# daigo0927/tf-raft

Measured on AMD Instinct MI355X. Metric: image-pairs/sec at 448×512 iters_pred=24; final-iter EPE vs TF ref, higher is better.
Workload: dtype f32; 1 GPU; RAFT forward BASELINE configs[1]: batch 4/GPU 448x512 iters_pred=24 random weights; pairs_per_gpu=4, global_batch=4, parallelism=dp1, collective=none

## Files before the change

### tf_raft_amd/csrc/conv_halo.h

```cpp
#pragma once
#include <stdlib.h>
#include <type_traits>

#include "conv_mfma.h"

template <int KH, int KW, int TH, int TN, int EPI, int STRIDE = 1, int PRE = 0, int STATS = 0, int STEM = 0, int DEEP = 0>
__global__ void __launch_bounds__(256) conv_halo_kernel(ConvArgs p) {
    constexpr int TW = 16, NKK = 2;
    constexpr int TAPS = KH * KW, R = TAPS * NKK;
    constexpr int LSTEP = (TAPS == 1 && !STEM) ? STRIDE : 1;
    constexpr int FSTEP = (TAPS == 1) ? 1 : STRIDE;
    constexpr int LDA = (FSTEP == 2) ? 36 : 40;
    constexpr int HH = (TH - 1) * FSTEP + KH, HWP = (TW - 1) * FSTEP + KW, HP = HH * HWP;
    constexpr int NA = (HP * 8 + 255) / 256;
    constexpr int A_BUF = HP * LDA + 8;
    constexpr int BN = 64 * TN;
    static_assert(!STEM || (TAPS == 1 && STRIDE == 2 && !PRE), "stem mode: 1x1 addressing, stride 2");
    __shared__ __attribute__((aligned(16))) float smem[2 * A_BUF];

    const int tid = threadIdx.x, lane = tid & 63, wn = tid >> 6;
    const int G = lane >> 4, LR = lane & 15;
    const int tiles_x = (p.W + TW - 1) / TW, tiles_y = (p.H + TH - 1) / TH;
    const int ntn = p.npad / BN;
    const int M = p.B * p.H * p.W;
    const int Hi = p.Hi, Wi = p.Wi;
    const int Min = p.B * Hi * Wi;

    int bid = blockIdx.x;
    {
        const int nwg = gridDim.x, xcd = bid & 7, q = nwg >> 3, r = nwg & 7;
        bid = (xcd < r ? xcd * (q + 1) : r * (q + 1) + (xcd - r) * q) + (bid >> 3);
    }
    const int mt = bid / ntn, nt = bid - mt * ntn;
    const int tx = mt % tiles_x, ty = (mt / tiles_x) % tiles_y, b = mt / (tiles_x * tiles_y);
    const int y0 = ty * TH, x0 = tx * TW;
    const int n0 = nt * BN;
    const int cin = p.c0 + p.c1;
    const int nch = cin >> 5;

    const __amdgpu_buffer_rsrc_t rs0 = __builtin_amdgcn_make_buffer_rsrc(
        (void *)p.a0, 0, (int)((((long)Min - 1) * p.lda0 + (STEM ? 4 : p.c0)) * 4), 0x00020000);
    const __amdgpu_buffer_rsrc_t rs1 = __builtin_amdgcn_make_buffer_rsrc(
        (void *)(p.c1 ? p.a1 : p.a0), 0, p.c1 ? (int)((((long)Min - 1) * p.lda1 + p.c1) * 4) : 0, 0x00020000);
    const __amdgpu_buffer_rsrc_t rsw = __builtin_amdgcn_make_buffer_rsrc(
        (void *)p.wp, 0, (int)((long)TAPS * cin * p.npad * 4), 0x00020000);

    int pix[NA];
    int lds_off[NA];
#pragma unroll
    for (int i = 0; i < NA; ++i) {
        const int item = tid + 256 * i;
        const int hp = item >> 3, c4 = item & 7;
        const int hy = hp / HWP, hx = hp - hy * HWP;
        lds_off[i] = hp < HP ? hp * LDA + c4 * 4 : HP * LDA;
        if (STEM) {
            const int yy = (y0 + hy) * 2 - p.pt, xx = (x0 + hx) * 2 - p.pl + c4;
            const bool ok = (hp < HP) & (c4 < 7) & ((unsigned)xx < (unsigned)Wi);
            pix[i] = ok ? (b * Hi + yy) * Wi + xx : -(1 << 30);
        } else {
            const int yy = y0 * STRIDE - p.pt + hy * LSTEP, xx = x0 * STRIDE - p.pl + hx * LSTEP;
            const bool ok = (hp < HP) & ((unsigned)yy < (unsigned)Hi) & ((unsigned)xx < (unsigned)Wi);
            pix[i] = ok ? (b * Hi + yy) * Wi + xx : -1;
        }
    }
    f32x4 ra[NA], pre_sc, pre_sh;
    auto gload = [&](int c) {
        if (STEM) {
#pragma unroll
            for (int i = 0; i < NA; ++i) {
                const int hp = (tid + 256 * i) >> 3;
                const int yy = (y0 + hp / HWP) * 2 - p.pt + c;
                const bool ok = (pix[i] > -(1 << 29)) & ((unsigned)yy < (unsigned)Hi);
                ra[i] = raft_buffer_load_f4(rs0, ok ? (unsigned)((pix[i] + c * Wi) * 16) : RAFT_OOB);
            }
            return;
        }
        const int ch = c * 32;
        const bool first = ch < p.c0;
        const int ld = first ? p.lda0 : p.lda1;
        const int chl = (first ? ch : ch - p.c0) + (tid & 7) * 4;
        if (first) {
#pragma unroll
            for (int i = 0; i < NA; ++i)
                ra[i] = raft_buffer_load_f4(rs0, pix[i] >= 0 ? (unsigned)((pix[i] * ld + chl) * 4) : RAFT_OOB);
        } else {
#pragma unroll
            for (int i = 0; i < NA; ++i)
                ra[i] = raft_buffer_load_f4(rs1, pix[i] >= 0 ? (unsigned)((pix[i] * ld + chl) * 4) : RAFT_OOB);
        }
        if (PRE) {
            pre_sc = *(const f32x4 *)(p.pre_scale + (long)b * cin + ch + (tid & 7) * 4);
            pre_sh = *(const f32x4 *)(p.pre_shift + (long)b * cin + ch + (tid & 7) * 4);
        }
    };
    auto lstore = [&](int buf) {
#pragma unroll
        for (int i = 0; i < NA; ++i) {
            f32x4 v = ra[i];
            if (PRE) {
#pragma unroll
                for (int e = 0; e < 4; ++e) v[e] = pix[i] >= 0 ? fmaxf(fmaf(v[e], pre_sc[e], pre_sh[e]), 0.f) : 0.f;
            }
            *(f32x4 *)(smem + buf * A_BUF + lds_off[i]) = v;
        }
    };

    f32x4 fa[2][TH], fb[DEEP ? 4 : 2][TN];
    const int a_lane = LR * FSTEP * LDA + G * 4;
    const unsigned b_lane = (unsigned)(((G * p.npad) + n0 + wn * 16 * TN + LR) * 16);
    auto frag_a = [&](int buf, int q, f32x4 *a) {
        const int t = q / NKK, kk = q - t * NKK;
        const float *base = smem + buf * A_BUF + a_lane + ((t / KW) * HWP + (t % KW)) * LDA + kk * 16;
#pragma unroll
        for (int i = 0; i < TH; ++i) a[i] = *(const f32x4 *)(base + i * FSTEP * HWP * LDA);
    };
    auto frag_b = [&](int c, int q, f32x4 *bf) {
        const int t = q / NKK, kk = q - t * NKK;
        const unsigned row = (unsigned)((t * (cin >> 2) + c * 8 + kk * 4) * p.npad) * 16u;
#pragma unroll
        for (int j = 0; j < TN; ++j)
            bf[j] = __builtin_bit_cast(f32x4, __builtin_amdgcn_raw_buffer_load_b128(rsw, (int)(b_lane + j * 256), (int)row, 0));
    };

    f32x4 acc[TH][TN];
#pragma unroll
    for (int i = 0; i < TH; ++i)
#pragma unroll
        for (int j = 0; j < TN; ++j) acc[i][j] = f32x4{0.f, 0.f, 0.f, 0.f};

    const int w0 = (EPI == EPI_GRU_ZR) ? p.hid : p.nvalid;
    const int w1 = (EPI == EPI_GRU_ZR) ? p.nvalid - p.hid : 0;
    const __amdgpu_buffer_rsrc_t ro0 = __builtin_amdgcn_make_buffer_rsrc(
        (void *)p.o0, 0, (int)((((long)M - 1) * p.ldo0 + w0) * 4), 0x00020000);
    const __amdgpu_buffer_rsrc_t ro1 = __builtin_amdgcn_make_buffer_rsrc(
        (void *)(w1 > 0 ? p.o1 : p.o0), 0, w1 > 0 ? (int)((((long)M - 1) * p.ldo1 + w1) * 4) : 0, 0x00020000);
    const bool has_e0 = EPI == EPI_GRU_ZR || EPI == EPI_GRU_Q || EPI == EPI_RES, has_e1 = EPI == EPI_GRU_Q;
    const int we = (EPI == EPI_GRU_ZR) ? p.hid : p.nvalid;
    const __amdgpu_buffer_rsrc_t re0 = __builtin_amdgcn_make_buffer_rsrc(
        (void *)(has_e0 ? (const void *)p.e0 : (const void *)p.o0), 0,
        has_e0 ? (int)((((long)M - 1) * p.lde0 + we) * 4) : 0, 0x00020000);
    const __amdgpu_buffer_rsrc_t re1 = __builtin_amdgcn_make_buffer_rsrc(
        (void *)(has_e1 ? (const void *)p.e1 : (const void *)p.o0), 0,
        has_e1 ? (int)((((long)M - 1) * p.lde1 + we) * 4) : 0, 0x00020000);
    auto bstore = [](float v, __amdgpu_buffer_rsrc_t r, unsigned off) {
        __builtin_amdgcn_raw_buffer_store_b32(__builtin_bit_cast(unsigned, v), r, (int)off, 0, 0);
    };
    auto bload = [](__amdgpu_buffer_rsrc_t r, unsigned off) {
        return __builtin_bit_cast(float, __builtin_amdgcn_raw_buffer_load_b32(r, (int)off, 0, 0));
    };
    float pe0[TH][TN][4], pe1[TH][TN][4];
    if (EPI == EPI_RES || EPI == EPI_GRU_ZR || EPI == EPI_GRU_Q) {
#pragma unroll
        for (int i = 0; i < TH; ++i)
#pragma unroll
            for (int j = 0; j < TN; ++j) {
                const int n = n0 + (wn * TN + j) * 16 + LR;
                const bool nok = n < p.nvalid;
                const bool isz = n < p.hid;
                const unsigned ne = (EPI == EPI_GRU_ZR) ? (unsigned)(isz ? n : n - p.hid) : (unsigned)n;
                const bool want0 = (EPI == EPI_GRU_ZR) ? (nok & !isz) : nok;
#pragma unroll
                for (int r = 0; r < 4; ++r) {
                    const int yy = y0 + i, xx = x0 + 4 * G + r;
                    const bool mokr = (yy < p.H) & (xx < p.W);
                    const unsigned m = (unsigned)((b * p.H + yy) * p.W + xx);
                    pe0[i][j][r] = bload(re0, (want0 & mokr) ? (m * p.lde0 + ne) * 4u : RAFT_OOB);
                    if (EPI == EPI_GRU_Q) pe1[i][j][r] = bload(re1, (nok & mokr) ? (m * p.lde1 + n) * 4u : RAFT_OOB);
                }
            }
    }
    gload(0);
    frag_b(0, 0, fb[0]);
    if (p.init) {
        const __amdgpu_buffer_rsrc_t ri = __builtin_amdgcn_make_buffer_rsrc(
            (void *)p.init, 0, (int)((((long)M - 1) * p.ldi + p.nvalid) * 4), 0x00020000);
#pragma unroll
        for (int i = 0; i < TH; ++i)
#pragma unroll
            for (int j = 0; j < TN; ++j) {
                const int n = n0 + (wn * TN + j) * 16 + LR;
#pragma unroll
                for (int r = 0; r < 4; ++r) {
                    const int yy = y0 + i, xx = x0 + 4 * G + r;
                    const bool ok = (yy < p.H) & (xx < p.W) & (n < p.nvalid);
                    const unsigned m = (unsigned)((b * p.H + yy) * p.W + xx);
                    acc[i][j][r] = __builtin_bit_cast(
                        float, __builtin_amdgcn_raw_buffer_load_b32(ri, ok ? (int)((m * p.ldi + n) * 4u) : (int)RAFT_OOB, 0, 0));
                }
            }
    }
    lstore(0);
    raft_barrier_lds();
    if (nch > 1) gload(1);
    frag_a(0, 0, fa[0]);
    if constexpr (DEEP) {
        static_assert(R % 2 == 0 && R >= 2, "ring indexing needs an even number of rounds per chunk");
        frag_b(0, 1, fb[1]);
        auto chunk = [&](auto parity, int c) {
            constexpr int P = decltype(parity)::value;
            const bool more = c + 1 < nch;
#pragma unroll
            for (int q = 0; q < R; ++q) {
                const int cur = q & 1;
                constexpr int RB = P * R;
                if (q + 1 < R)
                    frag_a(P, q + 1, fa[cur ^ 1]);
                else if (more)
                    frag_a(P ^ 1, 0, fa[cur ^ 1]);
                if (q + 2 < R)
                    frag_b(c, q + 2, fb[(RB + q + 2) & 3]);
                else if (more)
                    frag_b(c + 1, q + 2 - R, fb[(RB + q + 2) & 3]);
#pragma unroll
                for (int r = 0; r < 4; ++r)
#pragma unroll
                    for (int i = 0; i < TH; ++i)
#pragma unroll
                        for (int j = 0; j < TN; ++j)
                            acc[i][j] = __builtin_amdgcn_mfma_f32_16x16x4f32(fa[cur][i][r], fb[(RB + q) & 3][j][r], acc[i][j], 0, 0, 0);
                if (q == R - 2) {
                    if (more) {
                        lstore(P ^ 1);
                        if (c + 2 < nch) gload(c + 2);
                    }
                    raft_barrier_lds();
                }
            }
        };
        int c = 0;
        for (; c + 1 < nch; c += 2) {
            chunk(std::integral_constant<int, 0>{}, c);
            chunk(std::integral_constant<int, 1>{}, c + 1);
        }
        if (c < nch) chunk(std::integral_constant<int, 0>{}, c);
    } else
    for (int c = 0; c < nch; ++c) {
        const int buf = c & 1;
        const bool more = c + 1 < nch;
#pragma unroll
        for (int q = 0; q < R; ++q) {
            const int cur = q & 1;
            if (q + 1 < R) {
                frag_a(buf, q + 1, fa[cur ^ 1]);
                frag_b(c, q + 1, fb[cur ^ 1]);
            } else if (more) {
                frag_a(buf ^ 1, 0, fa[cur ^ 1]);
                frag_b(c + 1, 0, fb[cur ^ 1]);
            }
#pragma unroll
            for (int r = 0; r < 4; ++r)
#pragma unroll
                for (int i = 0; i < TH; ++i)
#pragma unroll
                    for (int j = 0; j < TN; ++j)
                        acc[i][j] = __builtin_amdgcn_mfma_f32_16x16x4f32(fa[cur][i][r], fb[cur][j][r], acc[i][j], 0, 0, 0);
            if (q == R - 2) {
                if (more) {
                    lstore(buf ^ 1);
                    if (c + 2 < nch) gload(c + 2);
                }
                raft_barrier_lds();
            }
        }
    }

    float biasv[TN], s1[TN], s2[TN];
#pragma unroll
    for (int j = 0; j < TN; ++j) {
        biasv[j] = p.bias[n0 + (wn * TN + j) * 16 + LR];
        s1[j] = 0.f;
        s2[j] = 0.f;
    }
#pragma unroll
    for (int i = 0; i < TH; ++i) {
        unsigned mrow[4];
        bool mok[4];
#pragma unroll
        for (int r = 0; r < 4; ++r) {
            const int yy = y0 + i, xx = x0 + 4 * G + r;
            mok[r] = (yy < p.H) & (xx < p.W);
            mrow[r] = (unsigned)((b * p.H + yy) * p.W + xx);
        }
#pragma unroll
        for (int j = 0; j < TN; ++j) {
            const int n = n0 + (wn * TN + j) * 16 + LR;
            const bool nok = n < p.nvalid;
            const float bias = biasv[j];
            if (EPI == EPI_LINEAR || EPI == EPI_RELU) {
#pragma unroll
                for (int r = 0; r < 4; ++r) {
                    float v = acc[i][j][r] + bias;
                    if (EPI == EPI_RELU) v = fmaxf(v, 0.f);
                    v *= p.scale;
                    if (STATS && mok[r]) {
                        s1[j] += v;
                        s2[j] = fmaf(v, v, s2[j]);
                    }
                    bstore(v, ro0, (nok & mok[r]) ? (mrow[r] * p.ldo0 + n) * 4u : RAFT_OOB);
                }
            } else if (EPI == EPI_RES) {
#pragma unroll
                for (int r = 0; r < 4; ++r)
                    bstore(fmaxf(pe0[i][j][r] + fmaxf(acc[i][j][r] + bias, 0.f), 0.f), ro0,
                           (nok & mok[r]) ? (mrow[r] * p.ldo0 + n) * 4u : RAFT_OOB);
            } else if (EPI == EPI_GRU_ZR) {
                const bool isz = n < p.hid;
                const unsigned nh = (unsigned)(isz ? n : n - p.hid);
#pragma unroll
                for (int r = 0; r < 4; ++r) {
                    const float g = raft_sigmoid(acc[i][j][r] + bias);
                    const bool ok = nok & mok[r];
                    bstore(g, ro0, (ok & isz) ? (mrow[r] * p.ldo0 + nh) * 4u : RAFT_OOB);
                    bstore(g * pe0[i][j][r], ro1, (ok & !isz) ? (mrow[r] * p.ldo1 + nh) * 4u : RAFT_OOB);
                }
            } else {
#pragma unroll
                for (int r = 0; r < 4; ++r) {
                    const float q = raft_tanh(acc[i][j][r] + bias);
                    bstore((1.0f - pe1[i][j][r]) * pe0[i][j][r] + pe1[i][j][r] * q, ro0,
                           (nok & mok[r]) ? (mrow[r] * p.ldo0 + n) * 4u : RAFT_OOB);
                }
            }
        }
    }
    if (STATS) {
#pragma unroll
        for (int j = 0; j < TN; ++j) {
            float a = s1[j], q = s2[j];
            a += __shfl_xor(a, 16, 64);
            q += __shfl_xor(q, 16, 64);
            a += __shfl_xor(a, 32, 64);
            q += __shfl_xor(q, 32, 64);
            const int n = n0 + (wn * TN + j) * 16 + LR;
            if (G == 0) *(float2 *)(p.stats + ((long)mt * p.npad + n) * 2) = make_float2(a, q);
        }
    }
}

int raft_launch_conv_halo_1x1(const ConvArgs &a, int th, int tn, int epi, hipStream_t s);
int raft_launch_conv_halo_3x3(const ConvArgs &a, int th, int tn, int epi, hipStream_t s);
int raft_launch_conv_halo_1x5(const ConvArgs &a, int th, int tn, int epi, hipStream_t s);
int raft_launch_conv_halo_5x1(const ConvArgs &a, int th, int tn, int epi, hipStream_t s);

static inline bool raft_conv_deep(const ConvArgs &, int, int tn, int) {
    return tn == 1;
}

template <int KH, int KW, int EPI>
static int raft_launch_conv_halo_tile(const ConvArgs &a, int th, int tn, hipStream_t s) {
    const int tiles = a.B * ((a.H + th - 1) / th) * ((a.W + 15) / 16);
    const int grid = tiles * (a.npad / (64 * tn));
    const int key = th * 10 + tn + (raft_conv_deep(a, th, tn, grid) ? 100 : 0);
    switch (key) {
        case 141: conv_halo_kernel<KH, KW, 4, 1, EPI, 1, 0, 0, 0, 1><<<grid, 256, 0, s>>>(a); break;
        case 171: conv_halo_kernel<KH, KW, 7, 1, EPI, 1, 0, 0, 0, 1><<<grid, 256, 0, s>>>(a); break;
        case 181: conv_halo_kernel<KH, KW, 8, 1, EPI, 1, 0, 0, 0, 1><<<grid, 256, 0, s>>>(a); break;
        case 41: conv_halo_kernel<KH, KW, 4, 1, EPI><<<grid, 256, 0, s>>>(a); break;
        case 42: conv_halo_kernel<KH, KW, 4, 2, EPI><<<grid, 256, 0, s>>>(a); break;
        case 71: conv_halo_kernel<KH, KW, 7, 1, EPI><<<grid, 256, 0, s>>>(a); break;
        case 72: conv_halo_kernel<KH, KW, 7, 2, EPI><<<grid, 256, 0, s>>>(a); break;
        case 81: conv_halo_kernel<KH, KW, 8, 1, EPI><<<grid, 256, 0, s>>>(a); break;
        case 82: conv_halo_kernel<KH, KW, 8, 2, EPI><<<grid, 256, 0, s>>>(a); break;
        default: return RAFT_E_UNSUPPORTED;
    }
    return raft_launch_status();
}

template <int KH, int KW>
static int raft_launch_conv_halo_epi(const ConvArgs &a, int th, int tn, int epi, hipStream_t s) {
    return raft_dispatch_epi<EPI_LINEAR, EPI_RELU, EPI_GRU_ZR, EPI_GRU_Q>(
        epi, [&](auto e) { return raft_launch_conv_halo_tile<KH, KW, decltype(e)::value>(a, th, tn, s); });
}
```

### tf_raft_amd/csrc/encoder.hip

```cpp
#include "conv_halo.h"
#include "conv_wino.h"

namespace {

__global__ void __launch_bounds__(256) enc_prep_kernel(const float *__restrict__ img, const float *__restrict__ img_b,
                                                       int64_t npix_a, f32x4 *__restrict__ out, int64_t npix, int affine) {
    const int64_t i = (int64_t)blockIdx.x * 256 + threadIdx.x;
    if (i >= npix) return;
    const float *src = i < npix_a ? img + 3 * i : img_b + 3 * (i - npix_a);
    float r = src[0], g = src[1], b = src[2];
    if (affine) {
#pragma clang fp contract(off)
        r = 2.f * (r / 255.f) - 1.f;
        g = 2.f * (g / 255.f) - 1.f;
        b = 2.f * (b / 255.f) - 1.f;
    }
    out[i] = f32x4{r, g, b, 0.f};
}

__global__ void __launch_bounds__(1024) in_finalize_kernel(const float *__restrict__ part, int tiles, int npad, int C,
                                                           const float *__restrict__ gamma, const float *__restrict__ beta,
                                                           double inv_count, float *__restrict__ scale,
                                                           float *__restrict__ shift) {
    __shared__ double sh[2][16][64];
    const int img = blockIdx.y, c = blockIdx.x * 64 + (threadIdx.x & 63), grp = threadIdx.x >> 6;
    double a = 0.0, q = 0.0;
    if (c < C) {
        const float2 *src = (const float2 *)part + ((int64_t)img * tiles) * npad + c;
        double a1 = 0.0, q1 = 0.0, a2 = 0.0, q2 = 0.0, a3 = 0.0, q3 = 0.0;
        int t = grp;
        for (; t + 48 < tiles; t += 64) {
            const float2 v0 = src[(int64_t)t * npad], v1 = src[(int64_t)(t + 16) * npad];
            const float2 v2 = src[(int64_t)(t + 32) * npad], v3 = src[(int64_t)(t + 48) * npad];
            a += (double)v0.x; q += (double)v0.y;
            a1 += (double)v1.x; q1 += (double)v1.y;
            a2 += (double)v2.x; q2 += (double)v2.y;
            a3 += (double)v3.x; q3 += (double)v3.y;
        }
        for (; t < tiles; t += 16) {
            const float2 v = src[(int64_t)t * npad];
            a += (double)v.x;
            q += (double)v.y;
        }
        a = (a + a1) + (a2 + a3);
        q = (q + q1) + (q2 + q3);
    }
    sh[0][grp][threadIdx.x & 63] = a;
    sh[1][grp][threadIdx.x & 63] = q;
    __syncthreads();
    if (grp == 0 && c < C) {
        for (int g = 1; g < 16; ++g) {
            a += sh[0][g][threadIdx.x];
            q += sh[1][g][threadIdx.x];
        }
        const double mean = a * inv_count;
        double var = q * inv_count - mean * mean;
        if (var < 0.0) var = 0.0;
        const double sc = (double)gamma[c] / sqrt(var + 1e-3);
        scale[(int64_t)img * C + c] = (float)sc;
        shift[(int64_t)img * C + c] = (float)((double)beta[c] - mean * sc);
    }
}

__global__ void __launch_bounds__(256) res_merge_kernel(const f32x4 *__restrict__ x, const float *__restrict__ xs,
                                                        const float *__restrict__ xh, const f32x4 *__restrict__ f,
                                                        const float *__restrict__ fs, const float *__restrict__ fh,
                                                        f32x4 *__restrict__ y, int64_t total4, int c4n, int64_t pix_per_img,
                                                        int mode) {
    const int64_t i = (int64_t)blockIdx.x * 256 + threadIdx.x;
    if (i >= total4) return;
    const int c4 = (int)(i % c4n);
    const int64_t img = (i / c4n) / pix_per_img;
    const f32x4 s = *(const f32x4 *)(fs + (img * c4n + c4) * 4), h = *(const f32x4 *)(fh + (img * c4n + c4) * 4);
    f32x4 v = f[i];
#pragma unroll
    for (int e = 0; e < 4; ++e) v[e] = fmaxf(fmaf(v[e], s[e], h[e]), 0.f);
    if (mode == 0) {
        f32x4 xv = x[i];
        if (xs) {
            const f32x4 s2 = *(const f32x4 *)(xs + (img * c4n + c4) * 4), h2 = *(const f32x4 *)(xh + (img * c4n + c4) * 4);
#pragma unroll
            for (int e = 0; e < 4; ++e) xv[e] = fmaf(xv[e], s2[e], h2[e]);
        }
#pragma unroll
        for (int e = 0; e < 4; ++e) v[e] = fmaxf(xv[e] + v[e], 0.f);
    }
    y[i] = v;
}

enum EncKind { ENC_3x3_S1, ENC_3x3_S2, ENC_1x1_S2, ENC_1x1_S1, ENC_STEM };

template <int KH, int KW, int EPI, int STRIDE, int PRE, int STATS, int STEM>
int launch_tile(const ConvArgs &a, int th, int tn, hipStream_t s) {
    const int tiles = a.B * ((a.H + th - 1) / th) * ((a.W + 15) / 16);
    const int grid = tiles * (a.npad / (64 * tn));
    const int key = th * 10 + tn + (raft_conv_deep(a, th, tn, grid) ? 100 : 0);
    switch (key) {
        case 171: conv_halo_kernel<KH, KW, 7, 1, EPI, STRIDE, PRE, STATS, STEM, 1><<<grid, 256, 0, s>>>(a); break;
        case 181: conv_halo_kernel<KH, KW, 8, 1, EPI, STRIDE, PRE, STATS, STEM, 1><<<grid, 256, 0, s>>>(a); break;
        case 71: conv_halo_kernel<KH, KW, 7, 1, EPI, STRIDE, PRE, STATS, STEM><<<grid, 256, 0, s>>>(a); break;
        case 72: conv_halo_kernel<KH, KW, 7, 2, EPI, STRIDE, PRE, STATS, STEM><<<grid, 256, 0, s>>>(a); break;
        case 81: conv_halo_kernel<KH, KW, 8, 1, EPI, STRIDE, PRE, STATS, STEM><<<grid, 256, 0, s>>>(a); break;
        case 82: conv_halo_kernel<KH, KW, 8, 2, EPI, STRIDE, PRE, STATS, STEM><<<grid, 256, 0, s>>>(a); break;
        default: return RAFT_E_UNSUPPORTED;
    }
    return raft_launch_status();
}

int enc_conv(const ConvArgs &a, EncKind kind, int epi, int th, int tn, hipStream_t s) {
    const bool pre = a.pre_scale != nullptr, stats = a.stats != nullptr;
    switch (kind) {
        case ENC_3x3_S1:
            if (epi == EPI_LINEAR && stats && !pre) return launch_tile<3, 3, EPI_LINEAR, 1, 0, 1, 0>(a, th, tn, s);
            if (epi == EPI_LINEAR && stats && pre) return launch_tile<3, 3, EPI_LINEAR, 1, 1, 1, 0>(a, th, tn, s);
            if (epi == EPI_RELU && !pre) return launch_tile<3, 3, EPI_RELU, 1, 0, 0, 0>(a, th, tn, s);
            if (epi == EPI_RES && !pre) return launch_tile<3, 3, EPI_RES, 1, 0, 0, 0>(a, th, tn, s);
            break;
        case ENC_3x3_S2:
            if (epi == EPI_LINEAR && stats && !pre) return launch_tile<3, 3, EPI_LINEAR, 2, 0, 1, 0>(a, th, tn, s);
            if (epi == EPI_RELU && !pre) return launch_tile<3, 3, EPI_RELU, 2, 0, 0, 0>(a, th, tn, s);
            break;
        case ENC_1x1_S2:
            if (epi == EPI_LINEAR && stats && !pre) return launch_tile<1, 1, EPI_LINEAR, 2, 0, 1, 0>(a, th, tn, s);
            if (epi == EPI_LINEAR && !stats && !pre) return launch_tile<1, 1, EPI_LINEAR, 2, 0, 0, 0>(a, th, tn, s);
            break;
        case ENC_1x1_S1:
            if (epi == EPI_LINEAR && !stats && !pre) return launch_tile<1, 1, EPI_LINEAR, 1, 0, 0, 0>(a, th, tn, s);
            break;
        case ENC_STEM:
            if (epi == EPI_LINEAR && stats) return launch_tile<1, 1, EPI_LINEAR, 2, 0, 1, 1>(a, th, tn, s);
            if (epi == EPI_RELU) return launch_tile<1, 1, EPI_RELU, 2, 0, 0, 1>(a, th, tn, s);
            break;
    }
    return RAFT_E_UNSUPPORTED;
}

void enc_pick(int H, int npad, int *th, int *tn) {
    *th = (H % 7 == 0) ? 7 : 8;
    *tn = 1;
    (void)npad;
}

void same_pad(int in, int k, int stride, int *out, int *before) {
    *out = (in + stride - 1) / stride;
    int total = (*out - 1) * stride + k - in;
    if (total < 0) total = 0;
    *before = total / 2;
}

struct EncBufs {
    float *img4, *x, *y, *r1, *r2, *rd, *part, *ss;
};

int64_t align4(int64_t v) { return (v + 3) & ~(int64_t)3; }

}

extern "C" int64_t raft_encoder_workspace_floats(const raft_encoder_weights *w, int n, int H, int W) {
    if (!w || n <= 0 || H <= 0 || W <= 0) return 0;
    const int64_t h1 = (H + 1) / 2, w1 = (W + 1) / 2;
    int cmax = w->c0 > w->c1 ? w->c0 : w->c1;
    if (w->c2 > cmax) cmax = w->c2;
    if (w->c3 > cmax) cmax = w->c3;
    const int64_t act = align4((int64_t)n * h1 * w1 * cmax);
    int64_t tiles = (int64_t)n * ((h1 + 6) / 7) * ((w1 + 15) / 16);
    const int64_t tiles_w = (int64_t)n * 2 * ((h1 + 3) / 4) * ((w1 + 31) / 32);
    if (tiles_w > tiles) tiles = tiles_w;
    const int64_t part = align4(tiles * 256 * 2);
    const int64_t ss = align4((int64_t)n * 256 * 2 * 3);
    return align4((int64_t)n * H * W * 4) + 5 * act + part + ss;
}

static int encoder_impl(const raft_encoder_weights *w, const float *images, const float *images_b, int n_a, int n, int H, int W,
                        int input_affine, float *out, float *workspace, void *stream, int hint);

extern "C" int raft_encoder_f32(const raft_encoder_weights *w, const float *images, int n, int H, int W,
                                int input_affine, float *out, float *workspace, void *stream) {
    return encoder_impl(w, images, images, n, n, H, W, input_affine, out, workspace, stream, raft_concurrency());
}

extern "C" int raft_encoder_pair_f32(const raft_encoder_weights *w, const float *images_a, const float *images_b, int n_each,
                                     int H, int W, int input_affine, float *out, float *workspace, void *stream) {
    RAFT_REQUIRE_PTR(images_b);
    RAFT_REQUIRE(n_each > 0, RAFT_E_SHAPE);
    return encoder_impl(w, images_a, images_b, n_each, 2 * n_each, H, W, input_affine, out, workspace, stream, raft_concurrency());
}

static int encoder_impl(const raft_encoder_weights *w, const float *images, const float *images_b, int n_a, int n, int H, int W,
                        int input_affine, float *out, float *workspace, void *stream, int hint) {
    RAFT_REQUIRE_PTR(w);
    RAFT_REQUIRE_PTR(images);
    RAFT_REQUIRE_PTR(out);
    RAFT_REQUIRE_PTR(workspace);
    RAFT_REQUIRE(n > 0 && H > 0 && W > 0, RAFT_E_SHAPE);
    RAFT_REQUIRE(w->c0 % 32 == 0 && w->c1 % 32 == 0 && w->c2 % 32 == 0 && w->c3 % 32 == 0, RAFT_E_UNSUPPORTED);
    RAFT_REQUIRE(w->c0 <= 256 && w->c1 <= 256 && w->c2 <= 256 && w->c3 <= 256 && w->cout > 0, RAFT_E_UNSUPPORTED);
    RAFT_REQUIRE(w->norm == RAFT_NORM_NONE || w->norm == RAFT_NORM_INSTANCE || w->norm == RAFT_NORM_FOLDED,
                 RAFT_E_UNSUPPORTED);
    RAFT_REQUIRE((int64_t)n * H * W * 4 * 4 < ((int64_t)1 << 31), RAFT_E_UNSUPPORTED);
    hipStream_t s = (hipStream_t)stream;
    const bool inorm = w->norm == RAFT_NORM_INSTANCE;

    const int64_t h1 = (H + 1) / 2, w1 = (W + 1) / 2;
    int cmax = w->c0 > w->c1 ? w->c0 : w->c1;
    if (w->c2 > cmax) cmax = w->c2;
    if (w->c3 > cmax) cmax = w->c3;
    const int64_t act = align4((int64_t)n * h1 * w1 * cmax);
    int64_t tiles_max = (int64_t)n * ((h1 + 6) / 7) * ((w1 + 15) / 16);
    {
        const int64_t tiles_w = (int64_t)n * 2 * ((h1 + 3) / 4) * ((w1 + 31) / 32);
        if (tiles_w > tiles_max) tiles_max = tiles_w;
    }
    const bool use_wino = raft_enc_wino();
    EncBufs b;
    float *p = workspace;
    b.img4 = p; p += align4((int64_t)n * H * W * 4);
    b.x = p; p += act;
    b.y = p; p += act;
    b.r1 = p; p += act;
    b.r2 = p; p += act;
    b.rd = p; p += act;
    b.part = p; p += align4(tiles_max * 256 * 2);
    b.ss = p;
    float *ss_slot[3][2];
    for (int k = 0; k < 3; ++k) {
        ss_slot[k][0] = b.ss + (int64_t)k * n * 256 * 2;
        ss_slot[k][1] = ss_slot[k][0] + (int64_t)n * 256;
    }

    {
        const int64_t npix = (int64_t)n * H * W;
        enc_prep_kernel<<<raft_ceil_div(npix, 256), 256, 0, s>>>(images, images_b, (int64_t)n_a * H * W, (f32x4 *)b.img4, npix, input_affine);
        RAFT_TRY(raft_launch_status());
    }

    auto conv = [&](EncKind kind, const raft_conv_weights &cw_direct, const float *in, int cin, int Hi, int Wi, int Ho, int Wo,
                    int pt, int pl, int cout, int epi, float *dst, const float *res, const float *pre_sc,
                    const float *pre_sh, int slot, const float *gamma, const float *beta,
                    const raft_conv_weights *cw_wino = nullptr, const raft_conv_weights *cw_wino4 = nullptr) -> int {
        const bool wino4 = kind == ENC_3x3_S1 && cw_wino4 && cw_wino4->wp != nullptr && cin % 16 == 0;
        const bool wino = !wino4 && use_wino && kind == ENC_3x3_S1 && cw_wino && cw_wino->wp != nullptr;
        const raft_conv_weights &cw = wino4 ? *cw_wino4 : (wino ? *cw_wino : cw_direct);
        ConvArgs a = {};
        a.a0 = in; a.lda0 = (kind == ENC_STEM) ? 4 : cin; a.c0 = (kind == ENC_STEM) ? 7 * 32 : cin;
        a.wp = cw.wp; a.bias = cw.bias; a.npad = cw.npad; a.nvalid = cout;
        a.B = n; a.H = Ho; a.W = Wo; a.Hi = Hi; a.Wi = Wi; a.pt = pt; a.pl = pl;
        a.scale = 1.0f; a.o0 = dst; a.ldo0 = cout;
        a.e0 = res; a.lde0 = cout;
        a.pre_scale = pre_sc; a.pre_shift = pre_sh;
        a.stats = (inorm && slot >= 0) ? b.part : nullptr;
        int th, tn;
        enc_pick(Ho, cw.npad, &th, &tn);
        const bool plain = pre_sc == nullptr && a.stats == nullptr;
        int rc = wino4  ? raft_launch_conv_wino4(a, epi, s, raft_wino4_plan(n, Ho, Wo, a.c0, a.c1, a.npad, plain, hint))
                 : wino ? raft_launch_conv_wino(a, epi, s, raft_wino_plan(n, Ho, Wo, a.c0, a.c1, a.npad, plain, hint))
                        : enc_conv(a, kind, epi, th, tn, s);
        if (rc != RAFT_OK) return rc;
        if (a.stats) {
            const int tiles = wino4  ? 2 * ((Ho + 7) / 8) * ((Wo + 63) / 64)
                              : wino ? 2 * ((Ho + 3) / 4) * ((Wo + 31) / 32)
                                     : ((Ho + th - 1) / th) * ((Wo + 15) / 16);
            dim3 grid((cout + 63) / 64, n);
            in_finalize_kernel<<<grid, 1024, 0, s>>>(b.part, tiles, cw.npad, cout, gamma, beta, 1.0 / ((double)Ho * Wo),
                                                     ss_slot[slot][0], ss_slot[slot][1]);
            rc = raft_launch_status();
        }
        return rc;
    };
    auto merge = [&](const float *x, const float *xs, const float *xh, const float *f, const float *fs, const float *fh,
                     float *y, int Ho, int Wo, int C, int mode) -> int {
        const int64_t total4 = (int64_t)n * Ho * Wo * C / 4;
        res_merge_kernel<<<raft_ceil_div(total4, 256), 256, 0, s>>>((const f32x4 *)x, xs, xh, (const f32x4 *)f, fs, fh,
                                                                    (f32x4 *)y, total4, C / 4, (int64_t)Ho * Wo, mode);
        return raft_launch_status();
    };

    int Hc, Wc, pt, pl;
    same_pad(H, 7, 2, &Hc, &pt);
    same_pad(W, 7, 2, &Wc, &pl);
    int C = w->c0;
    if (inorm) {
        RAFT_TRY(conv(ENC_STEM, w->conv1, b.img4, 0, H, W, Hc, Wc, pt, pl, C, EPI_LINEAR, b.r1, nullptr, nullptr, nullptr,
                          0, w->in_gamma[0], w->in_beta[0]));
        RAFT_TRY(merge(nullptr, nullptr, nullptr, b.r1, ss_slot[0][0], ss_slot[0][1], b.x, Hc, Wc, C, 1));
    } else {
        RAFT_TRY(conv(ENC_STEM, w->conv1, b.img4, 0, H, W, Hc, Wc, pt, pl, C, EPI_RELU, b.x, nullptr, nullptr, nullptr,
                          -1, nullptr, nullptr));
    }

    float *x = b.x, *y = b.y;
    const int widths[3] = {w->c1, w->c2, w->c3};
    for (int blk = 0; blk < 6; ++blk) {
        const int F = widths[blk / 2];
        const int stride = (blk == 2 || blk == 4) ? 2 : 1;
        const raft_conv_weights &c1 = w->block[blk][0], &c2 = w->block[blk][1], &cd = w->block[blk][2];
        int Ho = Hc, Wo = Wc, p1t = 1, p1l = 1;
        if (stride == 2) {
            same_pad(Hc, 3, 2, &Ho, &p1t);
            same_pad(Wc, 3, 2, &Wo, &p1l);
        }
        const EncKind k1 = stride == 2 ? ENC_3x3_S2 : ENC_3x3_S1;
        const int ni = 1 + blk * 3;
        const bool w4 = raft_enc_stage_wino4(blk / 2, n, Ho, Wo, F, hint);
        const raft_conv_weights *w44a = w4 ? &w->block_w44[blk][0] : nullptr, *w44b = w4 ? &w->block_w44[blk][1] : nullptr;
        if (inorm) {
            RAFT_TRY(conv(k1, c1, x, C, Hc, Wc, Ho, Wo, p1t, p1l, F, EPI_LINEAR, b.r1, nullptr, nullptr, nullptr, 0,
                              w->in_gamma[ni], w->in_beta[ni], &w->block_w[blk][0], w44a));
            RAFT_TRY(conv(ENC_3x3_S1, c2, b.r1, F, Ho, Wo, Ho, Wo, 1, 1, F, EPI_LINEAR, b.r2, nullptr, ss_slot[0][0],
                              ss_slot[0][1], 1, w->in_gamma[ni + 1], w->in_beta[ni + 1], &w->block_w[blk][1], w44b));
            if (stride == 2) {
                RAFT_REQUIRE(cd.wp != nullptr, RAFT_E_NULL);
                RAFT_TRY(conv(ENC_1x1_S2, cd, x, C, Hc, Wc, Ho, Wo, 0, 0, F, EPI_LINEAR, b.rd, nullptr, nullptr, nullptr, 2,
                                  w->in_gamma[ni + 2], w->in_beta[ni + 2]));
                RAFT_TRY(merge(b.rd, ss_slot[2][0], ss_slot[2][1], b.r2, ss_slot[1][0], ss_slot[1][1], y, Ho, Wo, F, 0));
            } else {
                RAFT_TRY(merge(x, nullptr, nullptr, b.r2, ss_slot[1][0], ss_slot[1][1], y, Ho, Wo, F, 0));
            }
        } else {
            RAFT_TRY(conv(k1, c1, x, C, Hc, Wc, Ho, Wo, p1t, p1l, F, EPI_RELU, b.r1, nullptr, nullptr, nullptr, -1, nullptr,
                              nullptr, &w->block_w[blk][0], w44a));
            const float *shortcut = x;
            if (stride == 2) {
                RAFT_REQUIRE(cd.wp != nullptr, RAFT_E_NULL);
                RAFT_TRY(conv(ENC_1x1_S2, cd, x, C, Hc, Wc, Ho, Wo, 0, 0, F, EPI_LINEAR, b.rd, nullptr, nullptr, nullptr, -1,
                                  nullptr, nullptr));
                shortcut = b.rd;
            }
            RAFT_TRY(conv(ENC_3x3_S1, c2, b.r1, F, Ho, Wo, Ho, Wo, 1, 1, F, EPI_RES, y, shortcut, nullptr, nullptr, -1,
                              nullptr, nullptr, &w->block_w[blk][1], w44b));
        }
        float *t = x; x = y; y = t;
        C = F; Hc = Ho; Wc = Wo;
    }
    return conv(ENC_1x1_S1, w->conv2, x, C, Hc, Wc, Hc, Wc, 0, 0, w->cout, EPI_LINEAR, out, nullptr, nullptr, nullptr, -1,
                nullptr, nullptr);
}
```

### tf_raft_amd/csrc/launch_plan.h

```cpp
#pragma once

#include <stdint.h>

#include "../../include/raft_hip.h"

enum RaftOptionId {
    RAFT_OPT_CONV_WINO, RAFT_OPT_SMALL_WINO, RAFT_OPT_GRU_WINO, RAFT_OPT_GRU_WINO4, RAFT_OPT_WINO_TNW, RAFT_OPT_WINO_SB,
    RAFT_OPT_WINO_CK, RAFT_OPT_WINO1D_TM,
    RAFT_OPT_LOOKUP_FUSED, RAFT_OPT_ONDEMAND_BLOCK, RAFT_OPT_ENC_WINO,
    RAFT_OPT_WINO_KS, RAFT_OPT_CONV_WINO4, RAFT_OPT_WINO4_KS, RAFT_OPT_MASK_FUSED, RAFT_OPT_ENC_WINO4, RAFT_OPT_CONVC2_KS, RAFT_OPT_CONVF2_KS,
    RAFT_OPT_EVENT_FENCE, RAFT_OPT_CORR_XCD, RAFT_OPT_CORR_POOL,
    RAFT_OPT_COUNT
};
int raft_opt(int id, int dflt);
bool raft_opt_is_set(int id);
int raft_opt_conv_tile(int npad, int taps, bool (*valid)(int code, int npad));

enum RaftConvFamily { RAFT_FAM_HALO, RAFT_FAM_WINO, RAFT_FAM_WINO1D, RAFT_FAM_WINO4 };
struct HaloPlan { int th, tn; };
struct WinoPlan { int tnw, sb, ck, ks; };
struct Wino1dPlan { int mo, tnw, tm, ck; };
struct Wino4Plan { int ks; };
struct ConvChoice { int family; HaloPlan halo; WinoPlan wino; Wino1dPlan wino1d; Wino4Plan wino4; const raft_conv_weights *wt; };
typedef const raft_conv_weights *RaftWeights;
static inline ConvChoice raft_choice(HaloPlan p, RaftWeights wt = nullptr) { ConvChoice c = {RAFT_FAM_HALO}; c.halo = p; c.wt = wt; return c; }
static inline ConvChoice raft_choice(WinoPlan p, RaftWeights wt = nullptr) { ConvChoice c = {RAFT_FAM_WINO}; c.wino = p; c.wt = wt; return c; }
static inline ConvChoice raft_choice(Wino1dPlan p, RaftWeights wt = nullptr) { ConvChoice c = {RAFT_FAM_WINO1D}; c.wino1d = p; c.wt = wt; return c; }
static inline ConvChoice raft_choice(Wino4Plan p, RaftWeights wt = nullptr) { ConvChoice c = {RAFT_FAM_WINO4}; c.wino4 = p; c.wt = wt; return c; }

static inline bool raft_halo_code_valid(int code, int npad) {
    const int th = (code - 100) / 10, tn = (code - 100) % 10;
    return code >= 100 && (th == 4 || th == 7 || th == 8) && (tn == 1 || tn == 2) && npad % (64 * tn) == 0;
}

static inline HaloPlan raft_halo_plan(int B, int H, int W, int npad, int kh, int kw, int hint) {
    int code = raft_opt_conv_tile(npad, kh * kw, raft_halo_code_valid);
    if (code < 100) {
        static const int ths[3] = {4, 7, 8};
        double best = 1e30;
        code = 141;
        for (int ti = 0; ti < 3; ++ti)
            for (int tn = 1; tn <= 2; ++tn) {
                const int th = ths[ti];
                if (npad % (64 * tn)) continue;
                const int64_t blocks = (int64_t)B * ((H + th - 1) / th) * ((W + 15) / 16) * (npad / (64 * tn)) * hint;
                const int64_t per_cu = (blocks + 255) / 256;
                const int lds = 2 * ((th + kh - 1) * (16 + kw - 1) * 40 + 8) * 4;
                int resident = 160 * 1024 / lds;
                const int reg_limit = (tn == 2 && th >= 7) ? 1 : (th >= 7 ? 2 : 3);
                if (resident > reg_limit) resident = reg_limit;
                const int64_t conc = per_cu < resident ? per_cu : resident;
                const double pen = conc >= 3 ? 1.0 : (conc == 2 ? 1.05 : 1.15);
                const double eff = (th == 4 && kh * kw > 1) ? 0.88 : 1.0;
                const double cost = (double)per_cu * th * 16 * 64 * tn * pen / eff;
                if (cost < best) {
                    best = cost;
                    code = 100 + th * 10 + tn;
                }
            }
    }
    return {(code - 100) / 10, (code - 100) % 10};
}

static inline WinoPlan raft_wino_plan(int B, int H, int W, int c0, int c1, int npad, bool plain, int hint) {
    const int tiles = B * ((H + 3) / 4) * ((W + 31) / 32);
    const int forced = raft_opt(RAFT_OPT_WINO_TNW, 0);
    int tnw = (npad % 64 == 0 && (int64_t)tiles * (npad / 64) * hint >= 512) ? 2 : 1;
    if (forced == 1 || (forced == 2 && npad % 64 == 0)) tnw = forced;
    const int grid = tiles * (npad / (32 * tnw));
    const int sb = raft_opt(RAFT_OPT_WINO_SB, (tnw == 2 || grid <= 512) ? 1 : 0) != 0;
    const bool ck2_ok = c0 % 32 == 0 && c1 % 32 == 0;
    const bool ck2 = ck2_ok && raft_opt(RAFT_OPT_WINO_CK, grid <= 512 ? 2 : 1) == 2;
    const int ks = raft_opt(RAFT_OPT_WINO_KS, (tnw == 1 && grid * hint <= 224) ? 2 : 1);
    if (ks == 2 && tnw == 1 && ck2_ok && plain) {
        const bool ck4 = c0 % 64 == 0 && c1 % 64 == 0 && raft_opt(RAFT_OPT_WINO_CK, 4) == 4;
        return {1, 1, ck4 ? 4 : 2, 2};
    }
    return {tnw, sb, (tnw == 1 && ck2) ? 2 : 1, 1};
}

constexpr bool RAFT_WINO1D_CK2_DEFAULT = true;

static inline int raft_wino1d_tiles(int B, int H, int W, int kh, int mo, int tm) {
    if (mo == 4) return kh == 5 ? B * ((H + 7) / 8) * ((W + 15) / 16) : B * ((H + 1) / 2) * ((W + 63) / 64);
    return kh == 5 ? B * ((H + 4 * tm - 1) / (4 * tm)) * ((W + 15) / 16) : B * ((H + 2 * tm - 1) / (2 * tm)) * ((W + 31) / 32);
}

static inline Wino1dPlan raft_wino1d_plan(int B, int H, int W, int c0, int c1, int npad, int kh, int mo, int hint) {
    const int forced = raft_opt(RAFT_OPT_WINO_TNW, 0);
    const int tiles = raft_wino1d_tiles(B, H, W, kh, mo, 2);
    int tnw = (npad % 64 == 0 && (int64_t)tiles * (npad / 64) * hint >= 400) ? 2 : 1;
    if (forced == 1 || (forced == 2 && npad % 64 == 0)) tnw = forced;
    if (mo == 4) return {4, tnw, 1, 2};
    const int tm_forced = raft_opt(RAFT_OPT_WINO1D_TM, 0);
    const bool ck2 = c0 % 32 == 0 && c1 % 32 == 0 && raft_opt(RAFT_OPT_WINO_CK, RAFT_WINO1D_CK2_DEFAULT ? 2 : 1) == 2;
    int tm = (int64_t)tiles * (npad / (32 * tnw)) * hint >= 400 ? 2 : 1;
    if (tm_forced == 1 || tm_forced == 2) tm = tm_forced;
    return {2, tnw, tm, ck2 ? 2 : 1};
}

static inline Wino4Plan raft_wino4_plan(int B, int H, int W, int c0, int c1, int npad, bool plain, int hint, int layer_ks = 0) {
    const int grid1 = B * ((H + 7) / 8) * ((W + 63) / 64) * (npad / 64);
    int ks = raft_opt(RAFT_OPT_WINO4_KS, (layer_ks == 1 || layer_ks == 2) ? layer_ks : (grid1 * hint < 128 ? 2 : 1));
    if (ks != 2 || c0 % 32 || c1 % 32 || !plain) ks = 1;
    return {ks};
}

constexpr int RAFT_GRU_WINO_DEFAULT = 15;
constexpr int RAFT_GRU_WINO4_DEFAULT = 15;
constexpr int RAFT_WINO_DEFAULT = 13;
constexpr int RAFT_SMALL_WINO_DEFAULT = 15;
static inline int raft_wino4_default_mask(int64_t m) {
    return m < 2 * 3584 ? 0 : (8 | (m >= 3 * 3584 ? 1 | 2 : 0) | (m >= 8 * 3584 ? 4 : 0));
}

struct BasicLoopPlan {
    bool lookup_fused, mask_fused;
    ConvChoice convc1, convc2, convf2, conv, gru[4], fh1_mask0, fh1, mask2;
};

static inline BasicLoopPlan raft_basic_loop_plan(const raft_basic_update_weights &wt, int B, int h, int w, bool stored_volume, int hint) {
    BasicLoopPlan p = {};
    const int64_t m = (int64_t)B * h * w * hint;
    p.lookup_fused = stored_volume && wt.convc1_f.wp != nullptr && raft_opt(RAFT_OPT_LOOKUP_FUSED, 1) != 0;
    p.mask_fused = raft_opt(RAFT_OPT_MASK_FUSED, m >= 2 * 3584 ? 1 : 0) != 0 && wt.mask2.wp != nullptr && wt.mask2.npad == 576;
    p.convc1 = raft_choice(raft_halo_plan(B, h, w, wt.convc1.npad, 1, 1, hint), &wt.convc1);
    p.mask2 = raft_choice(raft_halo_plan(B, h, w, wt.mask2.npad, 1, 1, hint), &wt.mask2);

    const int wino = raft_opt(RAFT_OPT_CONV_WINO, RAFT_WINO_DEFAULT), wino4 = raft_opt(RAFT_OPT_CONV_WINO4, raft_wino4_default_mask(m));
    auto conv3x3 = [&](int bit, const raft_conv_weights &direct, const raft_conv_weights &w2, const raft_conv_weights &w44, int c0,
                       int layer_ks) {
        if (w44.wp != nullptr && (wino4 & bit)) return raft_choice(raft_wino4_plan(B, h, w, c0, 0, w44.npad, true, hint, layer_ks), &w44);
        if ((wino & bit) && w2.wp != nullptr) return raft_choice(raft_wino_plan(B, h, w, c0, 0, w2.npad, true, hint), &w2);
        return raft_choice(raft_halo_plan(B, h, w, direct.npad, 3, 3, hint), &direct);
    };
    p.convc2 = conv3x3(1, wt.convc2, wt.convc2_w, wt.convc2_w44, 256, raft_opt(RAFT_OPT_CONVC2_KS, 0));
    const int f2_grid1 = B * ((h + 7) / 8) * ((w + 63) / 64);
    p.convf2 = conv3x3(2, wt.convf2, wt.convf2_w, wt.convf2_w44, 128, raft_opt(RAFT_OPT_CONVF2_KS, f2_grid1 * hint >= 56 ? 1 : 0));
    p.conv = conv3x3(4, wt.conv, wt.conv_w, wt.conv_w44, 256, 0);
    p.fh1_mask0 = conv3x3(8, wt.fh1_mask0, wt.fh1_mask0_w, wt.fh1_mask0_w44, 128, 0);
    const int n4 = wt.fh1_mask0_w44.npad > 0 ? wt.fh1_mask0_w44.npad : wt.fh1_w44.npad;
    const int n2 = (wt.fh1_mask0_w.npad > 0 && wt.fh1_mask0_w.npad % 32 == 0) ? wt.fh1_mask0_w.npad : wt.fh1_w.npad;
    p.fh1 = wt.fh1_w44.wp != nullptr && (wino4 & 8) ? raft_choice(raft_wino4_plan(B, h, w, 128, 0, n4, true, hint), &wt.fh1_w44)
                                                    : raft_choice(raft_wino_plan(B, h, w, 128, 0, n2, true, hint), &wt.fh1_w);

    const int gmask = raft_opt(RAFT_OPT_GRU_WINO, RAFT_GRU_WINO_DEFAULT);
    const int gmask4 = raft_opt(RAFT_OPT_GRU_WINO4, m < 2 * 3584 ? 0 : RAFT_GRU_WINO4_DEFAULT);
    const raft_conv_weights *gw[4][3] = {{&wt.gru_zr1, &wt.gru_zr1_w, &wt.gru_zr1_w4}, {&wt.gru_q1, &wt.gru_q1_w, &wt.gru_q1_w4},
                                         {&wt.gru_zr2, &wt.gru_zr2_w, &wt.gru_zr2_w4}, {&wt.gru_q2, &wt.gru_q2_w, &wt.gru_q2_w4}};
    for (int l = 0; l < 4; ++l) {
        const int bit = 1 << l, kh = l < 2 ? 1 : 5, kw = 6 - kh;
        if ((gmask4 & bit) && gw[l][2]->wp != nullptr)
            p.gru[l] = raft_choice(raft_wino1d_plan(B, h, w, 128, 128, gw[l][2]->npad, kh, 4, hint), gw[l][2]);
        else if ((gmask & bit) && gw[l][1]->wp != nullptr)
            p.gru[l] = raft_choice(raft_wino1d_plan(B, h, w, 128, 128, gw[l][1]->npad, kh, 2, hint), gw[l][1]);
        else
            p.gru[l] = raft_choice(raft_halo_plan(B, h, w, gw[l][0]->npad, kh, kw, hint), gw[l][0]);
    }
    return p;
}

static inline ConvChoice raft_gru_ctx_plan(const raft_basic_update_weights &wt, int pass, int B, int h, int w, int hint) {
    const raft_conv_weights &w4 = pass == 0 ? wt.gru_ctx1_w4 : wt.gru_ctx2_w4;
    const int kh = pass == 0 ? 1 : 5;
    if (w4.wp != nullptr && (raft_opt(RAFT_OPT_GRU_WINO4, RAFT_GRU_WINO4_DEFAULT) & (pass == 0 ? 1 : 4)))
        return raft_choice(raft_wino1d_plan(B, h, w, 128, 0, w4.npad, kh, 4, hint), &w4);
    const raft_conv_weights &wc = pass == 0 ? wt.gru_ctx1 : wt.gru_ctx2;
    return raft_choice(raft_halo_plan(B, h, w, wc.npad, kh, 6 - kh, hint), &wc);
}

struct SmallLoopPlan { ConvChoice convc1, convf2, conv, gru_zr, gru_q, fh1; };

static inline SmallLoopPlan raft_small_loop_plan(const raft_small_update_weights &wt, int B, int h, int w, int hint) {
    SmallLoopPlan p = {};
    const int mask = raft_opt(RAFT_OPT_SMALL_WINO, RAFT_SMALL_WINO_DEFAULT);
    auto conv3x3 = [&](int bit, const raft_conv_weights &direct, const raft_conv_weights &w2, int c0, int c1) {
        return (mask & bit) && w2.wp != nullptr ? raft_choice(raft_wino_plan(B, h, w, c0, c1, w2.npad, true, hint), &w2)
                                                : raft_choice(raft_halo_plan(B, h, w, direct.npad, 3, 3, hint), &direct);
    };
    p.convc1 = raft_choice(raft_halo_plan(B, h, w, wt.convc1.npad, 1, 1, hint), &wt.convc1);
    p.convf2 = raft_choice(raft_halo_plan(B, h, w, wt.convf2.npad, 3, 3, hint), &wt.convf2);
    p.conv = conv3x3(1, wt.conv, wt.conv_w, 128, 0);
    p.gru_zr = conv3x3(2, wt.gru_zr, wt.gru_zr_w, 96, 160);
    p.gru_q = conv3x3(4, wt.gru_q, wt.gru_q_w, 96, 160);
    p.fh1 = conv3x3(8, wt.fh1, wt.fh1_w, 96, 0);
    return p;
}

static inline bool raft_enc_wino() { return raft_opt(RAFT_OPT_ENC_WINO, 1) != 0; }
static inline bool raft_enc_stage_wino4(int stage, int n, int Ho, int Wo, int F, int hint) {
    const int mask = raft_enc_wino() ? raft_opt(RAFT_OPT_ENC_WINO4, 7) : 0;
    return ((mask >> stage) & 1) &&
           (raft_opt_is_set(RAFT_OPT_ENC_WINO4) || (int64_t)n * ((Ho + 7) / 8) * ((Wo + 63) / 64) * ((F + 63) / 64) * hint > 256);
}
```

Measured before the change: 388.4 image-pairs/s.

## Add cost-model tile-width planner and idle-wave early exit for encoder halo convs

Replaces the fixed encoder halo-conv tile choice (TN=1) with a planner that estimates per-CU work from LDS/register residency and picks TN in {1,2,4}, plus a deep-pipeline flag. It enables wider TN kernels, including deep variants, and allows a partial last N tile. A new IDLE template path lets waves whose output columns are all beyond nvalid skip the MFMA work. These waves still take part in the cooperative LDS loads and barriers, because the other waves in the block depend on them. The aim is to cut redundant reloading of the A halo per channel tile, at the cost of more register pressure and compile variants.

```diff
diff --git a/tf_raft_amd/csrc/conv_halo.h b/tf_raft_amd/csrc/conv_halo.h
--- a/tf_raft_amd/csrc/conv_halo.h
+++ b/tf_raft_amd/csrc/conv_halo.h
@@ -4,7 +4,8 @@
 
 #include "conv_mfma.h"
 
-template <int KH, int KW, int TH, int TN, int EPI, int STRIDE = 1, int PRE = 0, int STATS = 0, int STEM = 0, int DEEP = 0>
+template <int KH, int KW, int TH, int TN, int EPI, int STRIDE = 1, int PRE = 0, int STATS = 0, int STEM = 0, int DEEP = 0,
+          int IDLE = 0>
 __global__ void __launch_bounds__(256) conv_halo_kernel(ConvArgs p) {
     constexpr int TW = 16, NKK = 2;
     constexpr int TAPS = KH * KW, R = TAPS * NKK;
@@ -21,7 +22,7 @@
     const int tid = threadIdx.x, lane = tid & 63, wn = tid >> 6;
     const int G = lane >> 4, LR = lane & 15;
     const int tiles_x = (p.W + TW - 1) / TW, tiles_y = (p.H + TH - 1) / TH;
-    const int ntn = p.npad / BN;
+    const int ntn = (p.npad + BN - 1) / BN;
     const int M = p.B * p.H * p.W;
     const int Hi = p.Hi, Wi = p.Wi;
     const int Min = p.B * Hi * Wi;
@@ -170,6 +171,21 @@
             }
     }
     gload(0);
+    if constexpr (IDLE) {
+        if (__builtin_amdgcn_readfirstlane(n0 + wn * 16 * TN) >= p.nvalid) {
+            lstore(0);
+            raft_barrier_lds();
+            if (nch > 1) gload(1);
+            for (int c = 0; c < nch; ++c) {
+                if (c + 1 < nch) {
+                    lstore((c & 1) ^ 1);
+                    if (c + 2 < nch) gload(c + 2);
+                }
+                raft_barrier_lds();
+            }
+            return;
+        }
+    }
     frag_b(0, 0, fb[0]);
     if (p.init) {
         const __amdgpu_buffer_rsrc_t ri = __builtin_amdgcn_make_buffer_rsrc(
diff --git a/tf_raft_amd/csrc/encoder.hip b/tf_raft_amd/csrc/encoder.hip
--- a/tf_raft_amd/csrc/encoder.hip
+++ b/tf_raft_amd/csrc/encoder.hip
@@ -90,55 +90,77 @@
 
 enum EncKind { ENC_3x3_S1, ENC_3x3_S2, ENC_1x1_S2, ENC_1x1_S1, ENC_STEM };
 
+constexpr int enc_tn_max(EncKind kind) { return kind == ENC_STEM ? 1 : ((kind == ENC_1x1_S2 || kind == ENC_1x1_S1) ? 4 : 2); }
+
 template <int KH, int KW, int EPI, int STRIDE, int PRE, int STATS, int STEM>
-int launch_tile(const ConvArgs &a, int th, int tn, hipStream_t s) {
-    const int tiles = a.B * ((a.H + th - 1) / th) * ((a.W + 15) / 16);
-    const int grid = tiles * (a.npad / (64 * tn));
-    const int key = th * 10 + tn + (raft_conv_deep(a, th, tn, grid) ? 100 : 0);
+int launch_tile(const ConvArgs &a, EncHaloPlan pl, hipStream_t s) {
+    constexpr int TNMAX = STEM ? 1 : (KH * KW == 1 ? 4 : 2);
+    const int tiles = a.B * ((a.H + pl.th - 1) / pl.th) * ((a.W + 15) / 16);
+    const int grid = tiles * ((a.npad + 64 * pl.tn - 1) / (64 * pl.tn));
+    const int key = pl.th * 10 + pl.tn + (pl.deep ? 100 : 0);
+    if (pl.tn > TNMAX || (pl.tn == 1 && !pl.deep)) return RAFT_E_UNSUPPORTED;
     switch (key) {
         case 171: conv_halo_kernel<KH, KW, 7, 1, EPI, STRIDE, PRE, STATS, STEM, 1><<<grid, 256, 0, s>>>(a); break;
         case 181: conv_halo_kernel<KH, KW, 8, 1, EPI, STRIDE, PRE, STATS, STEM, 1><<<grid, 256, 0, s>>>(a); break;
-        case 71: conv_halo_kernel<KH, KW, 7, 1, EPI, STRIDE, PRE, STATS, STEM><<<grid, 256, 0, s>>>(a); break;
-        case 72: conv_halo_kernel<KH, KW, 7, 2, EPI, STRIDE, PRE, STATS, STEM><<<grid, 256, 0, s>>>(a); break;
-        case 81: conv_halo_kernel<KH, KW, 8, 1, EPI, STRIDE, PRE, STATS, STEM><<<grid, 256, 0, s>>>(a); break;
-        case 82: conv_halo_kernel<KH, KW, 8, 2, EPI, STRIDE, PRE, STATS, STEM><<<grid, 256, 0, s>>>(a); break;
-        default: return RAFT_E_UNSUPPORTED;
+        default:
+            if constexpr (TNMAX >= 2) {
+                switch (key) {
+                    case 72: conv_halo_kernel<KH, KW, 7, 2, EPI, STRIDE, PRE, STATS, STEM, 0, 1><<<grid, 256, 0, s>>>(a); break;
+                    case 82: conv_halo_kernel<KH, KW, 8, 2, EPI, STRIDE, PRE, STATS, STEM, 0, 1><<<grid, 256, 0, s>>>(a); break;
+                    case 172: conv_halo_kernel<KH, KW, 7, 2, EPI, STRIDE, PRE, STATS, STEM, 1, 1><<<grid, 256, 0, s>>>(a); break;
+                    case 182: conv_halo_kernel<KH, KW, 8, 2, EPI, STRIDE, PRE, STATS, STEM, 1, 1><<<grid, 256, 0, s>>>(a); break;
+                    default:
+                        if constexpr (TNMAX >= 4) {
+                            switch (key) {
+                                case 74: conv_halo_kernel<KH, KW, 7, 4, EPI, STRIDE, PRE, STATS, STEM, 0, 1><<<grid, 256, 0, s>>>(a); break;
+                                case 84: conv_halo_kernel<KH, KW, 8, 4, EPI, STRIDE, PRE, STATS, STEM, 0, 1><<<grid, 256, 0, s>>>(a); break;
+                                case 174: conv_halo_kernel<KH, KW, 7, 4, EPI, STRIDE, PRE, STATS, STEM, 1, 1><<<grid, 256, 0, s>>>(a); break;
+                                case 184: conv_halo_kernel<KH, KW, 8, 4, EPI, STRIDE, PRE, STATS, STEM, 1, 1><<<grid, 256, 0, s>>>(a); break;
+                                default: return RAFT_E_UNSUPPORTED;
+                            }
+                            break;
+                        }
+                        return RAFT_E_UNSUPPORTED;
+                }
+                break;
+            }
+            return RAFT_E_UNSUPPORTED;
     }
     return raft_launch_status();
 }
 
-int enc_conv(const ConvArgs &a, EncKind kind, int epi, int th, int tn, hipStream_t s) {
+int enc_conv(const ConvArgs &a, EncKind kind, int epi, EncHaloPlan pl, hipStream_t s) {
     const bool pre = a.pre_scale != nullptr, stats = a.stats != nullptr;
     switch (kind) {
         case ENC_3x3_S1:
-            if (epi == EPI_LINEAR && stats && !pre) return launch_tile<3, 3, EPI_LINEAR, 1, 0, 1, 0>(a, th, tn, s);
-            if (epi == EPI_LINEAR && stats && pre) return launch_tile<3, 3, EPI_LINEAR, 1, 1, 1, 0>(a, th, tn, s);
-            if (epi == EPI_RELU && !pre) return launch_tile<3, 3, EPI_RELU, 1, 0, 0, 0>(a, th, tn, s);
-            if (epi == EPI_RES && !pre) return launch_tile<3, 3, EPI_RES, 1, 0, 0, 0>(a, th, tn, s);
+            if (epi == EPI_LINEAR && stats && !pre) return launch_tile<3, 3, EPI_LINEAR, 1, 0, 1, 0>(a, pl, s);
+            if (epi == EPI_LINEAR && stats && pre) return launch_tile<3, 3, EPI_LINEAR, 1, 1, 1, 0>(a, pl, s);
+            if (epi == EPI_RELU && !pre) return launch_tile<3, 3, EPI_RELU, 1, 0, 0, 0>(a, pl, s);
+            if (epi == EPI_RES && !pre) return launch_tile<3, 3, EPI_RES, 1, 0, 0, 0>(a, pl, s);
             break;
         case ENC_3x3_S2:
-            if (epi == EPI_LINEAR && stats && !pre) return launch_tile<3, 3, EPI_LINEAR, 2, 0, 1, 0>(a, th, tn, s);
-            if (epi == EPI_RELU && !pre) return launch_tile<3, 3, EPI_RELU, 2, 0, 0, 0>(a, th, tn, s);
+            if (epi == EPI_LINEAR && stats && !pre) return launch_tile<3, 3, EPI_LINEAR, 2, 0, 1, 0>(a, pl, s);
+            if (epi == EPI_RELU && !pre) return launch_tile<3, 3, EPI_RELU, 2, 0, 0, 0>(a, pl, s);
             break;
         case ENC_1x1_S2:
-            if (epi == EPI_LINEAR && stats && !pre) return launch_tile<1, 1, EPI_LINEAR, 2, 0, 1, 0>(a, th, tn, s);
-            if (epi == EPI_LINEAR && !stats && !pre) return launch_tile<1, 1, EPI_LINEAR, 2, 0, 0, 0>(a, th, tn, s);
+            if (epi == EPI_LINEAR && stats && !pre) return launch_tile<1, 1, EPI_LINEAR, 2, 0, 1, 0>(a, pl, s);
+            if (epi == EPI_LINEAR && !stats && !pre) return launch_tile<1, 1, EPI_LINEAR, 2, 0, 0, 0>(a, pl, s);
             break;
         case ENC_1x1_S1:
-            if (epi == EPI_LINEAR && !stats && !pre) return launch_tile<1, 1, EPI_LINEAR, 1, 0, 0, 0>(a, th, tn, s);
+            if (epi == EPI_LINEAR && !stats && !pre) return launch_tile<1, 1, EPI_LINEAR, 1, 0, 0, 0>(a, pl, s);
             break;
         case ENC_STEM:
-            if (epi == EPI_LINEAR && stats) return launch_tile<1, 1, EPI_LINEAR, 2, 0, 1, 1>(a, th, tn, s);
-            if (epi == EPI_RELU) return launch_tile<1, 1, EPI_RELU, 2, 0, 0, 1>(a, th, tn, s);
+            if (epi == EPI_LINEAR && stats) return launch_tile<1, 1, EPI_LINEAR, 2, 0, 1, 1>(a, pl, s);
+            if (epi == EPI_RELU) return launch_tile<1, 1, EPI_RELU, 2, 0, 0, 1>(a, pl, s);
             break;
     }
     return RAFT_E_UNSUPPORTED;
 }
 
-void enc_pick(int H, int npad, int *th, int *tn) {
-    *th = (H % 7 == 0) ? 7 : 8;
-    *tn = 1;
-    (void)npad;
+EncHaloPlan enc_plan(EncKind kind, int n, int H, int W, int nvalid, int npad, int hint) {
+    const bool k3 = kind == ENC_3x3_S1 || kind == ENC_3x3_S2;
+    const int stride = (kind == ENC_3x3_S1 || kind == ENC_1x1_S1) ? 1 : 2;
+    return raft_enc_halo_plan(n, H, W, nvalid, npad, k3 ? 3 : 1, k3 ? 3 : 1, stride, kind == ENC_STEM ? 49 : (k3 ? 9 : 1), enc_tn_max(kind), hint);
 }
 
 void same_pad(int in, int k, int stride, int *out, int *before) {
@@ -249,12 +271,12 @@
         a.e0 = res; a.lde0 = cout;
         a.pre_scale = pre_sc; a.pre_shift = pre_sh;
         a.stats = (inorm && slot >= 0) ? b.part : nullptr;
-        int th, tn;
-        enc_pick(Ho, cw.npad, &th, &tn);
+        const EncHaloPlan hp = enc_plan(kind, n, Ho, Wo, cout, cw.npad, hint);
+        const int th = hp.th;
         const bool plain = pre_sc == nullptr && a.stats == nullptr;
         int rc = wino4  ? raft_launch_conv_wino4(a, epi, s, raft_wino4_plan(n, Ho, Wo, a.c0, a.c1, a.npad, plain, hint))
                  : wino ? raft_launch_conv_wino(a, epi, s, raft_wino_plan(n, Ho, Wo, a.c0, a.c1, a.npad, plain, hint))
-                        : enc_conv(a, kind, epi, th, tn, s);
+                        : enc_conv(a, kind, epi, hp, s);
         if (rc != RAFT_OK) return rc;
         if (a.stats) {
             const int tiles = wino4  ? 2 * ((Ho + 7) / 8) * ((Wo + 63) / 64)
diff --git a/tf_raft_amd/csrc/launch_plan.h b/tf_raft_amd/csrc/launch_plan.h
--- a/tf_raft_amd/csrc/launch_plan.h
+++ b/tf_raft_amd/csrc/launch_plan.h
@@ -193,3 +193,47 @@
     return ((mask >> stage) & 1) &&
            (raft_opt_is_set(RAFT_OPT_ENC_WINO4) || (int64_t)n * ((Ho + 7) / 8) * ((Wo + 63) / 64) * ((F + 63) / 64) * hint > 256);
 }
+
+struct EncHaloPlan { int th, tn, deep; };
+static inline bool raft_enc_code_valid(int code, int) {
+    const int tn = code % 10;
+    return code >= 100 && code < 300 && (tn == 1 || tn == 2 || tn == 4);
+}
+static inline EncHaloPlan raft_enc_halo_plan(int n, int H, int W, int nvalid, int npad, int kh, int kw, int stride, int key_taps,
+                                             int tn_max, int hint) {
+    const int th = (H % 7 == 0) ? 7 : 8;
+    const int fstep = kh * kw == 1 ? 1 : stride;
+    const int lds = 2 * (((th - 1) * fstep + kh) * (15 * fstep + kw) * (fstep == 2 ? 36 : 40) + 8) * 4;
+    const int by_lds = 160 * 1024 / lds;
+    const int64_t tiles = (int64_t)n * ((H + th - 1) / th) * ((W + 15) / 16);
+    auto resident = [&](int tn) {
+        const int by_regs = tn == 1 ? 3 : (tn == 2 ? 2 : 1);
+        return by_lds < by_regs ? by_lds : by_regs;
+    };
+    auto wgs = [&](int tn) { return (npad + 64 * tn - 1) / (64 * tn); };
+    auto per_cu = [&](int tn) { return (tiles * wgs(tn) * hint + 255) / 256; };
+    auto active = [&](int tn) { return tn == 1 ? 4 * wgs(1) : (nvalid + 16 * tn - 1) / (16 * tn); };
+    int tn = 1, deep = -1;
+    const int code = raft_opt_conv_tile(npad, key_taps, raft_enc_code_valid);
+    if (code >= 100 && code % 10 <= tn_max) {
+        tn = code % 10;
+        if (code >= 200 && tn > 1) deep = 0;
+    } else {
+        double best = 1e30;
+        for (int t = 1; t <= tn_max; t *= 2) {
+            double cost;
+            if (by_lds == 1) {
+                cost = (double)per_cu(t) * (32 * t + 18);
+            } else {
+                if (4 * wgs(t) - active(t) > 1) continue;
+                cost = (double)tiles * active(t) * hint / 1024.0 * (32 * t + (resident(t) == 1 ? 18 : 0));
+            }
+            if (cost < best) {
+                best = cost;
+                tn = t;
+            }
+        }
+    }
+    if (deep < 0) deep = (tn == 1 || per_cu(tn) == 1 || resident(tn) == 1) ? 1 : 0;
+    return {th, tn, deep};
+}
```

New measurement: 389.0 image-pairs/s (median of 6 runs). About the same (+0.2%).
